# Coda-Research-Group/LearnedMetricIndex

Measured on AMD Instinct MI355X. Metric: queries/sec @ recall@10, 768-d 10M index, 10k query batch, higher is better.
Workload: dtype f16 prefilter (f32 accumulate) + f32 exact re-rank; outputs identical to the all-f32 path

## Files before the change

### learnedmetricindex_amd/csrc/lmi_front.h

```cpp
#pragma once
#include "lmi_prefilter.h"

namespace lmi {

constexpr int FR_THREADS = 1024, FR_WAVES = FR_THREADS / 64;
constexpr int FR_MAX_L = 512;
constexpr int FR_MAX_SLOTS = 1 << 17;
constexpr int FR_SLICE_G = 48;
constexpr int FR_LIST = 512;
constexpr int FP_THREADS = 512, FP_WAVES = FP_THREADS / 64;
constexpr int FR_MAX_D = 64 * 4 * 8;
static_assert(FR_SLICE_G % 2 == 0, "the 16 x 32 fragment shape pairs k16-groups");

struct FrontParams {
    const int* bucket_order;
    int nq, nb, L;
    const unsigned* epoch_dev;
    unsigned long long* gran;
    int* cb_bucket;
    int* colmap;
    RouteArrays R;
    FillRanges Z;
    const float* q;
    int d, KG16, f16x16;
// ... 207 lines not shown
                const int p = (int)(ent & 0x7fffffffu);
                const int cpos = other ? n0 + c1 + (int)__popcll(bal1 & lt) : c0 + (int)__popcll(bal0 & lt);
                P.slot_col[p] = cbs * 32 + cpos;
                P.colmap[cbs * 32 + cpos] = p / nb;
            }
            c0 += (int)__popcll(bal0);
            c1 += (int)__popcll(bal1);
        }
    }
    FR_DBG(dbg_base, 2);
}

template <int GS, int CP, bool VEC>
__global__ __launch_bounds__(FP_THREADS) void pack_kernel(FrontParams P) {
    extern __shared__ __attribute__((aligned(16))) char fp_smem[];
    __shared__ int active_s;
    const int tid = threadIdx.x, lane = tid & 63, w = __builtin_amdgcn_readfirstlane(tid >> 6);
    const int bid = blockIdx.x;
    const unsigned epoch_v = *P.epoch_dev;
    for (int r = 0; r < P.Z.count; ++r)
        for (long long i = (long long)bid * FP_THREADS + tid; i < P.Z.n[r]; i += (long long)gridDim.x * FP_THREADS) P.Z.p[r][i] = P.Z.v[r];
    for (long long p = (long long)bid * FP_THREADS + tid; p < (long long)P.nq * P.nb; p += (long long)gridDim.x * FP_THREADS) {
        const int br = P.bucket_order[p];
        if (!(br >= 0 && br < P.L && P.R.nb_rows[br] > 0)) P.slot_col[p] = -1;
    }
    if (bid == 0) {
        FR_DBG(0, 0);
        const int L = P.L;
        int* nbr = reinterpret_cast<int*>(fp_smem);
        int* m_s = nbr + fr_lpad(L);
        int* m0_s = m_s + fr_lpad(L);
// ... 9 lines not shown
        for (int o = 32; o > 0; o >>= 1) { pairs += __shfl_xor(pairs, o); items += __shfl_xor(items, o); }
        __shared__ long long red[2][FP_WAVES];
        if (lane == 0) { red[0][w] = pairs; red[1][w] = items; }
        __syncthreads();
        if (tid == 0) {
            long long ps = 0, is = 0;
            for (int i = 0; i < FP_WAVES; ++i) { ps += red[0][i]; is += red[1][i]; }
            P.R.stats[0] = ps;
            P.R.stats[1] = is;
        }
        FR_DBG(0, 1);
        RouteArrays R2 = P.R;
        R2.m = m_s;
        R2.m0 = m0_s;
        R2.nb_rows = nbr;
        route_group_body<false, FP_THREADS>(L, R2, sort_s, &active_s);
        FR_DBG(0, 4);
        return;
    }
    const unsigned long long alloc = P.gran[P.L];
    const int n_cb = (unsigned)(alloc >> 32) == epoch_v ? (int)(unsigned)alloc : 0;
    const int cb = bid - 1;
    if (cb >= n_cb) return;
    char* stage = fp_smem;
    const int b = P.cb_bucket[cb];
    const int d = P.d, KG16 = P.KG16;
    const int nchunk_row = (d + 7) >> 3;
    constexpr int CPW = 64 / GS;
    constexpr int NCOL = (32 + FP_WAVES * CPW - 1) / (FP_WAVES * CPW);
    const int gl = lane % GS, sub = lane / GS;
    const float xn = __uint_as_float(P.bnorm[b]), dx = __uint_as_float(P.bdelta[b]);
// ... 101 lines not shown
```

### learnedmetricindex_amd/csrc/lmi_hip.hip

```cpp
#include "lmi_host.h"
#include "lmi_host_model.h"
#include "lmi_host_build.h"
#include "lmi_host_mutate.h"
#include "lmi_host_scan.h"
#include "lmi_host_search.h"
#include "lmi_host_comm.h"
#include "lmi_host_debug.h"
#include <mutex>

extern "C" LMI_API int lmi_abi_version(void) { return LMI_ABI_VERSION; }
#ifndef LMI_SOURCE_SHA16
#define LMI_SOURCE_SHA16 "unknown"
#endif
#define LMI_STR2(x) #x
#define LMI_STR(x) LMI_STR2(x)
extern "C" LMI_API const char* lmi_build_info(void) {
    return "src=" LMI_SOURCE_SHA16 " p2_waves=" LMI_STR(LMI_P2_WAVES) " p2_bring=" LMI_STR(LMI_P2_BR) " pf_cap=" LMI_STR(LMI_PF_CAP);
}
extern "C" LMI_API const char* lmi_last_error(void) { return g_err.c_str(); }

extern "C" LMI_API int lmi_create(int device, lmi_index** out) {
    if (!out) return fail("lmi_create: out is NULL");
    int ndev = 0;
    HIPCHK(hipGetDeviceCount(&ndev));
// ... 24 lines not shown
            HIPCHK(hipMemcpy(&ok, d_ok, sizeof(int), hipMemcpyDeviceToHost));
            HIPCHK(hipFree(d_ok));
            cached = ok;
        }
        h->pf_hw_ok = cached == 1;
        if (!h->pf_hw_ok) h->prefilter = false;
    }
    if (const char* e = getenv("LMI_RESCORE_SIMPLE")) h->rescore_streamed = !(e[0] && e[0] != '0');
    if (const char* e = getenv("LMI_PF_NO_REDO")) h->pf_redo = !(e[0] && e[0] != '0');
    if (const char* e = getenv("LMI_PF_SMALL")) h->pf_small = !(e[0] == '0');
    if (const char* e = getenv("LMI_PF_QBOUND")) h->pf_qbound = e[0] && e[0] != '0';
    if (const char* e = getenv("LMI_PF_PRIMARY")) h->pf_primary = e[0] && e[0] != '0';
    if (const char* e = getenv("LMI_PS_WIDE")) h->ps_force_wide = e[0] == '1' ? 1 : e[0] == '0' ? 0 : -1;
    if (const char* e = getenv("LMI_FRONT")) h->use_front = !(e[0] == '0');
    if (const char* e = getenv("LMI_P2_GRADED")) h->graded_chunks = !(e[0] == '0');
    if (const char* e = getenv("LMI_P2_CHUNKS")) (void)sscanf(e, "%d,%d,%d", &h->chunk_lvl_rows[0], &h->chunk_lvl_rows[1], &h->chunk_lvl_rows[2]);
    if (const char* e = getenv("LMI_P2_CHUNK_FRAC")) (void)sscanf(e, "%f,%f", &h->chunk_frac[0], &h->chunk_frac[1]);
    if (const char* e = getenv("LMI_TAIL")) h->use_tail = e[0] == '0' ? 0 : e[0] == '2' ? 2 : 1;
    if (const char* e = getenv("LMI_FR_DEBUG")) { if (e[0] == '1') { CHK(h->fr_dbg.reserve(256)); HIPCHK(hipMemset(h->fr_dbg.p, 0, 256)); } }
    {
        int khz = 0;
        if (hipDeviceGetAttribute(&khz, hipDeviceAttributeWallClockRate, device) == hipSuccess && khz > 0) h->wall_khz = (double)khz;
    }
#define LMI_PS_ATTR(K) \
    HIPCHK(hipFuncSetAttribute(reinterpret_cast<const void*>(&pass2_small_kernel<K, false, false>), hipFuncAttributeMaxDynamicSharedMemorySize, ps_lds_bytes(K, false))); \
    HIPCHK(hipFuncSetAttribute(reinterpret_cast<const void*>(&pass2_small_kernel<K, true, false>), hipFuncAttributeMaxDynamicSharedMemorySize, ps_lds_bytes(K, false))); \
    if constexpr (ps_has_wide(K)) { \
        HIPCHK(hipFuncSetAttribute(reinterpret_cast<const void*>(&pass2_small_kernel<K, false, ps_has_wide(K)>), hipFuncAttributeMaxDynamicSharedMemorySize, ps_lds_bytes(K, true))); \
        HIPCHK(hipFuncSetAttribute(reinterpret_cast<const void*>(&pass2_small_kernel<K, true, ps_has_wide(K)>), hipFuncAttributeMaxDynamicSharedMemorySize, ps_lds_bytes(K, true))); \
    }
// ... 103 lines not shown
```

### learnedmetricindex_amd/csrc/lmi_host.h

```cpp
#pragma once
#include "lmi_kernels.h"
#include "lmi_prefilter.h"
#include "lmi_pass2.h"
#include "lmi_pass2_small.h"
#include "lmi_mlp_fused.h"
#include "lmi_rescore.h"
#include "lmi_front.h"
#include "lmi_tail.h"
#include "lmi_mutate.h"

#include <algorithm>
#include <cfloat>
#include <cstdarg>
#include <cstdio>
#include <cstring>
#include <initializer_list>
#include <string>
#include <vector>

#include "lmi_hip.h"

using namespace lmi;

namespace {
// ... 136 lines not shown
    long long ev_calls = 0;
    hipEvent_t* ev = ev_ring[0];
    bool* ev_valid = valid_ring[0];
    long long h_stats[4] = {0, 0, 0, 0};
    bool stats_pending = false;
    DevBuf ts_ring;
    unsigned ts_mask[EV_RING] = {};
    unsigned long long* ts_set = nullptr;
    double wall_khz = 100000.0;
    DevBuf fr_dbg;
    DevBuf cb_alloc, cb_bucket;
    unsigned* h_oflag = nullptr;
    int overflow_armed = 0;
    bool fr_bump_pending = false;
    int use_tail = 1;
    bool graded_chunks = true;
    int chunk_lvl_rows[3] = {0, 0, 0};
    float chunk_frac[2] = {0.16f, 0.05f};
    bool use_front = true;

    std::vector<int> h_cap_rb;
    std::vector<unsigned char> h_owned;
    std::vector<unsigned char> h_any;
    lmi_index* parent = nullptr;
    int live_clones = 0;
    int64_t mut_paths[4] = {0, 0, 0, 0};
    DevBuf mut_pos, mut_ids, mut_list, mut_keep, mut_src, mut_stage, mut_word;
};

template <class F>
// ... 96 lines not shown
```

### learnedmetricindex_amd/csrc/lmi_host_debug.h

```cpp
#pragma once
#include "lmi_host_mutate.h"

static int read_event_set(const hipEvent_t* ev, const bool* ev_valid, float* ms) {
    for (int i = 0; i < LMI_T_COUNT; ++i) ms[i] = 0.0f;
    auto span = [&](int a, int b, float* out) -> int {
        if (ev_valid[a] && ev_valid[b]) HIPCHK(hipEventElapsedTime(out, ev[a], ev[b]));
        return 0;
    };
    CHK(span(0, 1, &ms[LMI_T_INFERENCE]));
    CHK(span(1, 2, &ms[LMI_T_ROUTE]));
    CHK(span(2, 3, &ms[LMI_T_SCAN]));
    CHK(span(3, 4, &ms[LMI_T_MERGE]));
    CHK(span(2, 5, &ms[LMI_T_PF_SAMPLE]));
    CHK(span(5, 6, &ms[LMI_T_PF_EMIT]));
    CHK(span(6, 7, &ms[LMI_T_RESCORE]));
    CHK(span(7, 3, &ms[LMI_T_FALLBACK]));
    int first = ev_valid[0] ? 0 : 1;
    int last = ev_valid[4] ? 4 : 1;
    CHK(span(first, last, &ms[LMI_T_TOTAL]));
    return 0;
}

static void read_stamp_set(const lmi_index* h, const unsigned long long* v, unsigned mask, float* ms) {
    for (int i = 0; i < LMI_T_COUNT; ++i) ms[i] = 0.0f;
// ... 144 lines not shown
    if (!strcmp(name, "pf_bound")) b = &h->pf_bound;
    if (!strcmp(name, "fr_dbg")) b = &h->fr_dbg;
    if (!strcmp(name, "pf_stamps")) { b = &h->pf_bound; off = h->stamps_off; }
    if (!strcmp(name, "cand_total")) {
        if (bytes != 8 || !h->last_fast) return fail("lmi_debug_peek: cand_total is 8 bytes after a prefilter scan");
        unsigned long long* d_acc = reinterpret_cast<unsigned long long*>(h->stats.as<long long>() + 2);
        HIPCHK(hipMemsetAsync(d_acc, 0, 8, h->stream));
        sum_u32_kernel<<<64, 256, 0, h->stream>>>(h->cand_cnt.as<unsigned>(), h->last_ncols, d_acc);
        HIPCHK(hipGetLastError());
        HIPCHK(hipStreamSynchronize(h->stream));
        HIPCHK(hipMemcpy(dst, d_acc, 8, hipMemcpyDeviceToHost));
        return 0;
    }
    if (!strcmp(name, "pf_redo")) b = &h->redo;
    if (!strcmp(name, "pf_fallback")) b = &h->fb_list;
    if (!b) return fail("lmi_debug_peek: unknown buffer '%s'", name);
    if (bytes < 0 || off + (size_t)bytes > b->cap) return fail("lmi_debug_peek: %lld bytes asked of a %zu-byte buffer", (long long)bytes, b->cap);
    if (bytes) HIPCHK(hipMemcpy(dst, static_cast<char*>(b->p) + off, (size_t)bytes, hipMemcpyDeviceToHost));
    return 0;
}

extern "C" LMI_API int lmi_scan_stats(lmi_index* h, double* flops, int64_t* pairs, int64_t* items) {
    if (!h) return fail("lmi_scan_stats: NULL handle");
    CHK(set_dev(h));
    if (h->stats_pending) {
        HIPCHK(hipStreamSynchronize(h->stream));
        HIPCHK(hipMemcpy(h->h_stats, h->stats.p, 32, hipMemcpyDeviceToHost));
        h->stats_pending = false;
    }
    if (pairs) *pairs = h->h_stats[0];
// ... 5 lines not shown
```

### learnedmetricindex_amd/csrc/lmi_host_scan.h

```cpp
#pragma once
#include "lmi_host.h"

static bool rescore_is_streamed(const lmi_index* h) {
    return h->rescore_streamed && rc_waves_for(h->dp, 4) > 0 && rc_wave_lds(h->dp, 4, true) <= RC_SMALL_LDS_CAP;
}
static int rescore_group_size(int nb) { return nb % 4 == 0 ? 4 : nb % 3 == 0 ? 3 : nb % 2 == 0 ? 2 : 1; }

struct ScanPlan {
    int nq, nb, kout, L;
    long long nslots;
    long long ncb_bound;
    long long ncols;
    int max_nch;
    long long part_lists;
    bool fast;
    bool low_d;
    bool ps_wide;
    int tile_cb;
    int sample_max;
    bool qbound;
    int primary_nb;
    bool use_front;
    bool streamed;
    int G, groups, sub_cap;
// ... 77 lines not shown
    augment_norm_kernel<<<cdiv(nq, 256), 256, 0, h->stream>>>(d_qs, h->d_user, h->d, nq, h->q_aug.as<float>(), h->qn2.as<float>());
    HIPCHK(hipGetLastError());
    C.q = h->q_aug.as<float>();
    C.qn2 = h->qn2.as<float>();
    return 0;
}

static int scan_reserve(lmi_index* h, ScanCall& C) {
    const ScanPlan& P = C.P;
    const int L = P.L;
    const size_t nslots = (size_t)P.nslots, ncols = (size_t)P.ncols;
    CHK(h->m.reserve((size_t)L * 4 * 3));
    CHK(h->cb_start.reserve((L + 1) * 4));
    CHK(h->item_base.reserve((L + 1) * 4));
    CHK(h->part_base.reserve((L + 1) * 8));
    CHK(h->stats.reserve(32));
    CHK(h->head.reserve(256));
    const size_t grp_ints = (size_t)NGRP * L + 2 * (size_t)NGRP * (L + 1) + 3 * NGRP + (size_t)L;
    CHK(h->grp.reserve(grp_ints * 4));
    CHK(h->slot_local.reserve(nslots * 4));
    CHK(h->slot_col.reserve(nslots * 4));
    CHK(h->colmap.reserve(ncols * 4));
    CHK(h->col_thr.reserve(ncols * 4));
    CHK(h->qfrag.reserve((size_t)P.ncb_bound * h->KGs * 1024));
    CHK(h->part_score.reserve((size_t)P.part_lists * KPB * 4));
    CHK(h->part_row.reserve((size_t)P.part_lists * KPB * 4));
    CHK(h->rank_d.reserve(nslots * KPB * 4));
    CHK(h->rank_id.reserve(nslots * KPB * 4));

    FillRanges& Z = C.Z;
    Z.count = 0;
// ... 60 lines not shown
    R.grp_base1 = R.grp_total + NGRP;
    R.grp_total1 = R.grp_base1 + (size_t)NGRP * (L + 1);
    R.dbg = nullptr;
    R.chunk_rb = h->chunk_rows / 32;
    R.chunk_rb_b = (P.fast && h->graded_chunks) ? R.grp_total1 + NGRP : nullptr;
    const int base = h->chunk_rows;
    int rows[3] = {base, base / 2, base / 4};
    if (P.low_d) rows[0] = 2 * base;
    for (int i = 0; i < 3; ++i) {
        if (h->chunk_lvl_rows[i] > 0) rows[i] = h->chunk_lvl_rows[i];
        rows[i] = std::max(P2_TILE_ROWS, rows[i] / P2_TILE_ROWS * P2_TILE_ROWS);
        R.chunk_lvl[i] = rows[i] / 32;
    }
    R.chunk_frac[0] = h->chunk_frac[0];
    R.chunk_frac[1] = h->chunk_frac[1];
    R.tile_cb = P.tile_cb;
    R.sample_max = P.sample_max;
    R.sample_items = P.fast ? 1 : 0;
    R.primary_nb = P.primary_nb;
}

static int front_separate(lmi_index* h, ScanCall& C) {
    const ScanPlan& P = C.P;
    const RouteArrays& R = C.R;
    const int L = P.L, nslots = (int)P.nslots;
    C.Z.ts = tsp(h, ST_FRONT);
    fill_ranges_kernel<<<h->num_cus * 4, 256, 0, h->stream>>>(C.Z);
    HIPCHK(hipGetLastError());
    route_count_kernel<<<cdiv(nslots, 256), 256, 0, h->stream>>>(C.order, nslots, L, R, h->slot_local.as<int>());
    HIPCHK(hipGetLastError());
// ... 124 lines not shown
    if (S.ts_start) { S.ts_end_cell = scan_end_cell(h); (void)tsp(h, ST_SCAN1); }
    scan_kernel<<<h->num_cus * h->scan_blocks_per_cu, 256, SCAN_LDS, h->stream>>>(S);
    HIPCHK(hipGetLastError());
    CHK(record(h, 3));
    return 0;
}

static void prefilter_params(lmi_index* h, const ScanCall& C, PrefilterParams& F) {
    const RouteArrays& R = C.R;
    F.slab16 = h->slab16.as<uint4>();
    F.qfrag16 = h->qfrag16.as<uint4>();
    F.KG16 = h->KG16;
    F.L = C.P.L;
    F.chunk_rb = R.chunk_rb;
    F.chunk_rb_b = R.chunk_rb_b;
    F.tile_cb = R.tile_cb;
    F.sample_max = R.sample_max;
    F.rb_start = h->d_rb_start.as<int>();
    F.nb_rows = R.nb_rows;
    F.nch = R.nch;
    F.m = R.m;
    F.m0 = R.m0;
    F.cb_start = R.cb_start;
    F.grp_bucket = R.grp_bucket;
    F.grp_base = R.grp_base;
    F.grp_n = R.grp_n;
    F.grp_total = R.grp_total;
    F.grp_base1 = R.grp_base1;
    F.grp_total1 = R.grp_total1;
    F.ncols = C.P.ncols;
// ... 279 lines not shown
```

### learnedmetricindex_amd/csrc/lmi_kernels.h

```cpp
#pragma once
#include <hip/hip_runtime.h>
#include <stdint.h>

namespace lmi {

typedef float f32x16 __attribute__((ext_vector_type(16)));

constexpr int KPB = 10;
#ifndef LMI_SCAN_RB
#define LMI_SCAN_RB 1
#endif
constexpr int RB = LMI_SCAN_RB;
constexpr int TILE_ROWS = 128 * RB;
constexpr int TILE_COLS = 128;
constexpr int STAGE_G = 4;
constexpr int SCAN_LDS = 0;
constexpr unsigned NOROW = 0xFFFFFFFFu;
constexpr int NGRP = 8;

__device__ __forceinline__ int acc_row(int r, int h) { return (r & 3) + 8 * (r >> 2) + 4 * h; }

enum { ST_MLP0 = 0, ST_MLP1, ST_FRONT, ST_P1, ST_P2, ST_P2END, ST_TAIL, ST_FB, ST_MERGE, ST_END, ST_SCAN0, ST_SCAN1,
       ST_CLK_WALL, ST_CLK_CYC,
       ST_COUNT = 16 };
// ... 313 lines not shown
    int* grp_bucket;
    int* grp_base;
    int* grp_n;
    int* grp_total;
    int* grp_base1;
    int* grp_total1;
    int tile_cb;
    int primary_nb;
    int sample_items;
    int sample_max;
    unsigned long long* dbg;
    int* chunk_rb_b;
    int chunk_rb;
    int chunk_lvl[3];
    float chunk_frac[2];
};
__device__ __forceinline__ int chunks_of(int n_rows, int crb) { return (((n_rows + 31) >> 5) + crb - 1) / crb; }

#ifndef LMI_PF_SAMPLE_ROWS
#define LMI_PF_SAMPLE_ROWS 512
#endif
#ifndef LMI_PF_SAMPLE
#define LMI_PF_SAMPLE 16
#endif
constexpr int PF_SAMPLE = LMI_PF_SAMPLE;
#ifndef LMI_PF_SAMPLE_LOWD
#define LMI_PF_SAMPLE_LOWD 8
#endif
constexpr int PF_SAMPLE_LOWD = LMI_PF_SAMPLE_LOWD, PF_SAMPLE_LOWD_KG = 4;
__device__ __forceinline__ int sample_stride(int n_b, int smax) {
// ... 23 lines not shown
    }
    local -= g_all * nqt_all;
    const int g = local / nqt_primary;
    *qt = local - g * nqt_primary;
    *j0 = g * P1_TPI * 2 + 1;
    *nt = min(P1_TPI, n_pri - g * P1_TPI);
    return false;
}
__device__ __forceinline__ int sample_tiles256(int n_b, int smax) {
    const int nt = (((n_b + 31) >> 5) + 7) / 8;
    const int s = sample_stride(n_b, smax);
    return (nt + s - 1) / s;
}

__device__ __forceinline__ int query_tiles(int m, int tile_cb) { return (((m + 31) >> 5) + tile_cb - 1) / tile_cb; }

constexpr int ROUTE_LDS_BUCKETS = 4096;
constexpr int ROUTE_OTHER = 1 << 30;
__global__ __launch_bounds__(256) void route_count_kernel(const int* __restrict__ bucket_order, int nslots, int L,
                                                          RouteArrays R, int* __restrict__ slot_local) {
    __shared__ int cnt_s[2 * ROUTE_LDS_BUCKETS];
    const int p = blockIdx.x * blockDim.x + threadIdx.x;
    int b = -1;
    bool other = false;
    if (p < nslots) {
        b = bucket_order[p];
        if (!(b >= 0 && b < L && R.nb_rows[b] > 0)) b = -1;
        if (b >= 0 && R.primary_nb > 0) {
            const int r = p % R.primary_nb;
            for (int j = p - r; j < p; ++j) {
// ... 67 lines not shown
}

__host__ __device__ inline int route_group_pow2(int L) { int p = 64; while (p < L) p <<= 1; return p; }
__host__ __device__ inline size_t route_group_lds(int L) { return (size_t)route_group_pow2(L) * 8 + (size_t)L * 8; }
constexpr int ROUTE_MAX_BUCKETS = 8000;
constexpr int ROUTE_ID_BITS = 20;
template <bool GLOBAL, int NT = 1024>
__device__ __forceinline__ void route_group_body(int L, const RouteArrays& R, char* base, int* active_sp) {
    int& active_s = *active_sp;
    const int P = route_group_pow2(L);
    unsigned long long* key_s = reinterpret_cast<unsigned long long*>(base);
    int* items_s = reinterpret_cast<int*>(key_s + P);
    int* items1_s = items_s + L;
    int* order_s = GLOBAL ? items1_s + L : reinterpret_cast<int*>(base);
    const int t = threadIdx.x;
    if (t == 0) active_s = 0;
    __syncthreads();
    {
        int mine = 0;
        for (int b = t; b < P; b += NT) {
            unsigned long long key = ~0ull;
            if (b < L) {
                const int m = R.m[b];
                long long work = (long long)m * R.nb_rows[b];
                mine += work > 0;
                items_s[b] = query_tiles(m, R.tile_cb) * R.nch[b];
                const int mp = R.sample_items ? R.m0[b] : 0;
                items1_s[b] = (R.sample_items && m > 0) ? pass1_items(sample_tiles256(R.nb_rows[b], R.sample_max), query_tiles(m, R.tile_cb), query_tiles(mp, R.tile_cb)) : 0;
                if (work > (1ll << 43) - 1) work = (1ll << 43) - 1;
                key = ((unsigned long long)((1ll << 43) - 1 - work) << ROUTE_ID_BITS) | (unsigned long long)b;
            }
            key_s[b] = key;
        }
        if (mine) atomicAdd(&active_s, mine);
    }
    __syncthreads();
    if (R.dbg && t == 0) R.dbg[2] = wall_clock64();
    bool ranked = false;
    int my_rank[2] = {0, 0}, my_id[2] = {0, 0};
    if (!GLOBAL && P <= 2 * NT && P <= 1024) {
        ranked = true;
#pragma unroll
        for (int u = 0; u < 2; ++u) {
            const int i = t + u * NT;
            if (i < P) {
                const unsigned long long mine = key_s[i];
                int r = 0;
                long long w_all = 0, w_tail = 0;
#pragma unroll 8
                for (int o = 0; o < P; ++o) {
                    const unsigned long long ko = key_s[o];
// ... 91 lines not shown
                        R.grp_base1[g * (L + 1) + r + 1] = carry + x;
                    }
                }
                carry += __shfl(x, 63, 64);
            }
            if (ln == 0) {
                if (!second) { R.grp_n[g] = n_g; R.grp_total[g] = carry; }
                else R.grp_total1[g] = carry;
            }
        }
    }
}
template <bool GLOBAL>
__global__ __launch_bounds__(1024) void route_group_kernel(int L, RouteArrays R, char* scratch) {
    extern __shared__ __attribute__((aligned(16))) char grp_smem[];
    __shared__ int active_s;
    route_group_body<GLOBAL>(L, R, GLOBAL ? scratch : grp_smem, &active_s);
}

__global__ void route_fill_kernel(const int* __restrict__ bucket_order, const int* __restrict__ slot_local,
                                  int nslots, int nb, const int* __restrict__ cb_start, const int* __restrict__ m0,
                                  int* __restrict__ colmap, int* __restrict__ slot_col) {
    int p = blockIdx.x * blockDim.x + threadIdx.x;
    if (p >= nslots) return;
    int loc = slot_local[p];
    int col = -1;
    if (loc >= 0) {
        const int b = bucket_order[p];
        col = cb_start[b] * 32 + ((loc & ROUTE_OTHER) ? m0[b] + (loc & (ROUTE_OTHER - 1)) : loc);
        colmap[col] = p / nb;
    }
    slot_col[p] = col;
// ... 521 lines not shown
```

### learnedmetricindex_amd/csrc/lmi_pass2.h

```cpp
#pragma once
#include <type_traits>

#include "lmi_prefilter.h"

namespace lmi {

constexpr int P2_G = 2;
constexpr int P2_MAXCB = 12;
#ifndef LMI_P2_WAVES
#define LMI_P2_WAVES 8
#endif
constexpr int P2_WAVES = LMI_P2_WAVES;
static_assert(P2_WAVES == 4 || P2_WAVES == 8, "");
constexpr int P2_BLOCKS_PER_CU = 8 / P2_WAVES;
constexpr int P2_TILE_RB = 8;
constexpr int P2_TILE_ROWS = 32 * P2_TILE_RB;
constexpr int P2_SLOT_BYTES = P2_MAXCB * P2_G * 1024;
constexpr int P2_RING = 3;
constexpr int P2_NSL = 16;
constexpr int P2_NSL_BIG = 8;
static_assert(P2_NSL * 16 == P2_NSL_BIG * 32, "bound_merge2_kernel reads 256 values per column either way");
constexpr int P2_LIST = 64 + 1;
constexpr int P2_AREG0 = 232;
#define LMI_P2_NUM_VGPR_ATTR 116
// ... 15 lines not shown

#ifdef LMI_P2_STAMPS
#ifndef LMI_P2_STAMPS_SAMPLE
#define LMI_P2_STAMPS_SAMPLE 0
#endif
#define P2_STAMP(PH) if (SAMPLE == (LMI_P2_STAMPS_SAMPLE != 0)) { const unsigned long long t_ = __builtin_readcyclecounter(); st_acc[PH] += t_ - st_last; st_last = t_; }
#else
#define P2_STAMP(PH)
#endif
#if defined(LMI_P2_STAMPS) && defined(LMI_P2_STAMPS_FINE)
#define P2_STAMP_FINE(PH) P2_STAMP(PH)
#else
#define P2_STAMP_FINE(PH)
#endif

template <int NCB, bool SAMPLE>
struct Tile2 {
    static constexpr int G = P2_G;
    static constexpr int Q = G * NCB;
#ifndef LMI_P2_BR
#define LMI_P2_BR 3
#endif
    static constexpr int BR = LMI_P2_BR;
    static_assert(BR == 3 || BR == 6, "3 Q must be a multiple of BR for every NCB");
    static constexpr int D = NCB < BR - 1 ? NCB : BR - 1;
    static constexpr int PBL = (NCB + 1) / 2;
    static constexpr int PA = G;
    static_assert(G == 2, "written out for two k-groups per stage");

    const PrefilterParams& P;
    unsigned ring;
    uint4* ring_p;
    uint2* sList;
    float* sThr;
    uint4* sPend;
    int lane, w;
    unsigned lds_lane;
    typedef float f32x4v __attribute__((ext_vector_type(4)));
    f32x4v acc[NCB][2][2];
// ... 168 lines not shown
        else asm volatile("s_waitcnt vmcnt(%1)" : "+v"(pend_pos) : "n"(2 * PA) : "memory");
        if (pend_pos != 0xffffffffu) {
            u32x4 e;
            const unsigned pa = (unsigned)reinterpret_cast<uintptr_t>(sPend + w * 64) + (unsigned)ln * 16u;
            asm volatile("ds_read_b128 %0, %1\n\ts_waitcnt lgkmcnt(0)" : "=v"(e) : "v"(pa) : "memory");
            cand_store(P, (size_t)e.x, pend_pos, e.y, __uint_as_float(e.z));
        }
        pend_pos = 0xffffffffu;
    }

    __device__ __forceinline__ void epilogue_emit(int rb_tile0, int n_b, size_t col0) {
        const int ln = lane_id();
        const int quad = ln >> 4, c16 = ln & 15;
#ifdef LMI_ABL_NOEPI
#pragma unroll
        for (int n = 0; n < NCB; ++n) asm volatile("" :: "v"(acc[n][0][0]), "v"(acc[n][1][0]), "v"(acc[n][0][1]), "v"(acc[n][1][1]));
        return;
#endif
        const unsigned row0 = (unsigned)((rb_tile0 + w) * 32);
        if (row0 + 32u > (unsigned)n_b) {
            int lim = n_b - (int)row0 - 4 * quad;
#pragma unroll
            for (int n = 0; n < NCB; ++n) {
                asm volatile("" : "+v"(lim));
#pragma unroll
                for (int rh = 0; rh < 2; ++rh)
#pragma unroll
                    for (int r = 0; r < 4; ++r)
                        if (16 * rh + r >= lim) { acc[n][rh][0][r] = __builtin_nanf(""); acc[n][rh][1][r] = __builtin_nanf(""); }
            }
        }
        const unsigned list_addr = (unsigned)reinterpret_cast<uintptr_t>(sList + w * P2_LIST);
        int tot = 0;
        const unsigned kb = (unsigned)((c16 << 8) | (4 * quad));
        const unsigned thr_addr = (unsigned)reinterpret_cast<uintptr_t>(sThr) + (unsigned)c16 * 4u;
        constexpr int TB = 2;
        float thr[2][TB][2];
        auto thr_load = [&](int nb0, float (&t)[TB][2]) __attribute__((always_inline)) {
#pragma unroll
            for (int i = 0; i < TB; ++i) {
                const int n = min(nb0 + i, NCB - 1);
                asm volatile("ds_read_b32 %0, %1" : "=v"(t[i][0]) : "v"(thr_addr + (unsigned)(n * 128)) : "memory");
                asm volatile("ds_read_b32 %0, %1" : "=v"(t[i][1]) : "v"(thr_addr + (unsigned)(n * 128 + 64)) : "memory");
            }
        };
        thr_load(0, thr[0]);
#pragma unroll
        for (int n = 0; n < NCB; ++n) {
            constexpr int dummy = 0; (void)dummy;
            if (n % TB == 0) {
                asm volatile("s_waitcnt lgkmcnt(0)" ::: "memory");
#pragma unroll
                for (int i = 0; i < TB; ++i) asm volatile("" : "+v"(thr[(n / TB) & 1][i][0]), "+v"(thr[(n / TB) & 1][i][1]));
                if (n + TB < NCB) thr_load(n + TB, thr[((n / TB) + 1) & 1]);
            }
            float gm[2][2], t0, mh[2];
#pragma unroll
            for (int ch = 0; ch < 2; ++ch) {
#pragma unroll
                for (int rh = 0; rh < 2; ++rh) {
                    asm("v_max3_f32 %0, %1, %2, %3" : "=v"(t0) : "v"(acc[n][rh][ch][0]), "v"(acc[n][rh][ch][1]), "v"(acc[n][rh][ch][2]));
                    asm("v_max_f32 %0, %1, %2" : "=v"(gm[ch][rh]) : "v"(t0), "v"(acc[n][rh][ch][3]));
                }
                asm("v_max_f32 %0, %1, %2" : "=v"(mh[ch]) : "v"(gm[ch][0]), "v"(gm[ch][1]));
            }
            const float th0 = thr[(n / TB) & 1][n % TB][0], th1 = thr[(n / TB) & 1][n % TB][1];
            bool any = (mh[0] >= th0) | (mh[1] >= th1);
#ifdef LMI_ABL_NOEMIT
            any = any && th0 == 12345.678f;
#endif
            if (__builtin_expect(__ballot(any) == 0ull, 1)) continue;
#pragma unroll
            for (int ch = 0; ch < 2; ++ch) {
                const float th = ch ? th1 : th0;
#pragma unroll
                for (int rh = 0; rh < 2; ++rh) {
                    if (__ballot(gm[ch][rh] >= th) == 0ull) continue;
#pragma unroll
                    for (int r = 0; r < 4; ++r) {
                        const bool pass = acc[n][rh][ch][r] >= th;
                        const unsigned long long mask = __ballot(pass);
                        if (__builtin_expect(mask != 0ull, 0)) {
                            if (pass) {
                                const int my = tot + (int)__builtin_amdgcn_mbcnt_hi((unsigned)(mask >> 32), __builtin_amdgcn_mbcnt_lo((unsigned)mask, 0u));
                                const unsigned key = kb + (unsigned)(((n * 32 + 16 * ch) << 8) | (16 * rh + r));
                                const unsigned la = list_addr + (unsigned)min(my, 64) * 8u;
                                const unsigned sb = __float_as_uint(acc[n][rh][ch][r]);
                                const u32x2 ent = {key, sb};
// ... 16 lines not shown
                const unsigned pa = (unsigned)reinterpret_cast<uintptr_t>(sPend + w * 64) + (unsigned)ln * 16u;
                asm volatile("ds_write_b128 %0, %1" :: "v"(pa), "v"(pe) : "memory");
#ifdef LMI_ABL_NOATOMIC
                pend_pos = (unsigned)ln;
#else
                const unsigned* cnt_addr = P.cand_cnt + pcol;
                const unsigned one = 1u;
                asm volatile("global_atomic_add %0, %1, %2, off sc0" : "=v"(pend_pos) : "v"(cnt_addr), "v"(one) : "memory");
#endif
            }
        } else if (tot > 64) {
#pragma unroll
            for (int n = 0; n < NCB; ++n) {
#pragma unroll
                for (int ch = 0; ch < 2; ++ch) {
                    const float th = sThr[n * 32 + 16 * ch + c16];
                    unsigned rowq = row0 + 4u * (unsigned)quad;
                    asm volatile("" : "+v"(rowq));
#pragma unroll
                    for (int rh = 0; rh < 2; ++rh)
#pragma unroll
                        for (int r = 0; r < 4; ++r)
                            if (acc[n][rh][ch][r] >= th) {
                                const size_t col = col0 + n * 32 + 16 * ch + c16;
                                const unsigned pos = atomicAdd(P.cand_cnt + col, 1u);
                                cand_store(P, col, pos, rowq + (unsigned)(16 * rh + r), acc[n][rh][ch][r]);
                            }
                }
            }
        }
// ... 1 lines not shown

    __device__ __forceinline__ void epilogue_sample(int rb_tile0, int n_b, size_t col0, int m_left, int list_j, bool use_atomic, int rb_in_tile) {
        const int ln = lane_id();
        const int quad = ln >> 4, c16 = ln & 15;
        const unsigned row0 = (unsigned)((rb_tile0 + w) * 32);
        const bool ragged = row0 + 32u > (unsigned)n_b;
        int lim = ragged ? n_b - (int)row0 - 4 * quad : 64;
#pragma unroll
        for (int n = 0; n < NCB; ++n) {
            if (ragged) {
                asm volatile("" : "+v"(lim));
#pragma unroll
                for (int rh = 0; rh < 2; ++rh)
#pragma unroll
                    for (int r = 0; r < 4; ++r)
                        if (16 * rh + r >= lim) { acc[n][rh][0][r] = -INFINITY; acc[n][rh][1][r] = -INFINITY; }
            }
#pragma unroll
            for (int ch = 0; ch < 2; ++ch) {
                float m0, m1, m2;
                asm("v_max3_f32 %0, %1, %2, %3" : "=v"(m0) : "v"(acc[n][0][ch][0]), "v"(acc[n][0][ch][1]), "v"(acc[n][0][ch][2]));
                asm("v_max3_f32 %0, %1, %2, %3" : "=v"(m1) : "v"(acc[n][1][ch][0]), "v"(acc[n][1][ch][1]), "v"(acc[n][1][ch][2]));
                asm("v_max3_f32 %0, %1, %2, %3" : "=v"(m2) : "v"(m0), "v"(m1), "v"(acc[n][0][ch][3]));
                asm("v_max_f32 %0, %1, %2" : "=v"(m2) : "v"(m2), "v"(acc[n][1][ch][3]));
                const float mx = m2;
                if (n * 32 + 16 * ch + c16 < m_left) {
                    float* dst = P.bound + ((size_t)(list_j * 32 + (rb_in_tile + w) * 4 + quad)) * (size_t)P.ncols + (col0 + n * 32 + 16 * ch + c16);
                    if (!use_atomic) *dst = mx;
                    else {
                        if (mx >= 0.0f) atomicMax(reinterpret_cast<int*>(dst), __float_as_int(mx));
                        else atomicMin(reinterpret_cast<unsigned*>(dst), __float_as_uint(mx));
                    }
                }
            }
// ... 176 lines not shown
    const int q = blockIdx.x * blockDim.x + threadIdx.x;
    if (q >= nq) return;
    float lq = -INFINITY;
    for (int r = 0; r < nb; ++r) {
        const int col = slot_col[q * nb + r];
        if (col >= 0) lq = fmaxf(lq, bound1[col] - 0.5f * eps2[col]);
    }
    if (!(lq > -INFINITY)) return;
    lq -= fabsf(lq) * 4.8e-7f;
    for (int r = 0; r < nb; ++r) {
        const int col = slot_col[q * nb + r];
        if (col >= 0) bound1[col] = fmaxf(bound1[col], lq + 0.5f * eps2[col] * 0.9999f);
    }
}

struct P2Item { int b, cbt0, ncb_tile, ch, m_use, nt; };
template <bool SAMPLE>
__device__ __forceinline__ void p2_decode_item(const PrefilterParams& P, int b, int local, P2Item& it) {
    int qt = 0, ch = 0, nt = 1;
    bool all_cols = true;
    if (SAMPLE) {
        const int nqa = query_tiles(P.m[b], P.tile_cb), nqp = query_tiles(P.m0[b], P.tile_cb);
        all_cols = pass1_decode(local, p2_sample_tiles(P.nb_rows[b], P.sample_max), nqa, nqp, &ch, &nt, &qt);
    }
    it.nt = nt;
    it.m_use = all_cols ? P.m[b] : P.m0[b];
    const int ncb_b = (it.m_use + 31) >> 5;
    const int nqt = (ncb_b + P.tile_cb - 1) / P.tile_cb;
    const int per = (ncb_b + nqt - 1) / nqt;
    if (!SAMPLE) { qt = local % nqt; ch = local / nqt; }
    it.b = b;
    it.ch = ch;
    it.cbt0 = qt * per;
    it.ncb_tile = min(per, ncb_b - it.cbt0);
}
template <bool SAMPLE>
__device__ __forceinline__ bool p2_pop_item(const PrefilterParams& P, int& grp, int* s_item, P2Item& it) {
    if (threadIdx.x == 0) {
        int b = -1, local = 0;
        do {
            b = -1;
            unsigned* heads = P.head + (SAMPLE ? 24 : 0);
            const int* totals = SAMPLE ? P.grp_total1 : P.grp_total;
            const int* bases = SAMPLE ? P.grp_base1 : P.grp_base;
            for (int tries = 0; tries < NGRP; ++tries) {
                const int tot = totals[grp];
                if (__hip_atomic_load(&heads[grp], __ATOMIC_RELAXED, __HIP_MEMORY_SCOPE_AGENT) < (unsigned)tot) {
                    const int itn = (int)atomicAdd(&heads[grp], 1u);
                    if (itn < tot) {
// ... 97 lines not shown
    __shared__ uint2 sList[SAMPLE ? 1 : P2_WAVES * P2_LIST];
    __shared__ float sThr[SAMPLE ? 1 : P2_MAXCB * 32];
    __shared__ __attribute__((aligned(16))) uint4 sPend[SAMPLE ? 1 : P2_WAVES * 64];
    __shared__ int s_item[2];
    __shared__ int s_prefix[P2_PREFIX_CAP_K];
    __shared__ int s_gb[P2_PREFIX_CAP_K];
    if (!SAMPLE && P.redo_count && *P.redo_count == 0u) return;
    ts_first(P.ts_start);
    unsigned long long clk_w0 = 0, clk_c0 = 0;
    if (!SAMPLE) clk_begin(P.ts_end_cell ? P.ts_start : nullptr, clk_w0, clk_c0);
    P2Queue<SAMPLE, 2, 64 * P2_WAVES, P2_PREFIX_CAP_K> queue{P, s_item, s_prefix, s_gb};
    queue.init();
    P2Item item;
    while (queue.next(item)) {
        const int b = item.b, cbt0 = item.cbt0, ch = item.ch, m_use = item.m_use, nt = item.nt;
#define P2_CASE(N) case N: { Tile2<N, SAMPLE> it{P, (unsigned)reinterpret_cast<uintptr_t>(ring), ring, sList, sThr, sPend}; it.run(b, cbt0, ch, m_use, nt, queue); break; }
        switch (item.ncb_tile) {
            P2_CASE(1) P2_CASE(2) P2_CASE(3) P2_CASE(4) P2_CASE(5) P2_CASE(6)
            P2_CASE(7) P2_CASE(8) P2_CASE(9) P2_CASE(10) P2_CASE(11)
            default: { Tile2<12, SAMPLE> it{P, (unsigned)reinterpret_cast<uintptr_t>(ring), ring, sList, sThr, sPend}; it.run(b, cbt0, ch, m_use, nt, queue); break; }
        }
#undef P2_CASE
    }
    if (!SAMPLE) clk_end(P.ts_end_cell ? P.ts_start : nullptr, ST_P2, clk_w0, clk_c0);
#ifdef LMI_P2_ENDS
    if (!SAMPLE && P.ts_end_cell && threadIdx.x == 0 && blockIdx.x < 256) {
        P.stamps[192 + blockIdx.x] = wall_clock64();
        if (blockIdx.x == 0) P.stamps[191] = clk_w0;
    }
#endif
    ts_max(P.ts_end_cell);
}

}
```

### learnedmetricindex_amd/csrc/lmi_prefilter.h

```cpp
#pragma once
#include "lmi_kernels.h"


namespace lmi {

typedef _Float16 half8 __attribute__((ext_vector_type(8)));

constexpr int PF_STAGE_G = 2;
#ifndef LMI_PF_CAP
#define LMI_PF_CAP 1024
#endif
constexpr int PF_CAP = LMI_PF_CAP;
constexpr int PF_KEEP = 64;

__global__ void scatter_rows_kernel(const float* __restrict__ src, int d, const int* __restrict__ pos,
                                    long long row0, const long long* __restrict__ index, long long n_total, long long nrows,
                                    float* __restrict__ dst, int pitch) {
    const long long idx = (long long)blockIdx.x * blockDim.x + threadIdx.x;
    if (idx >= nrows * d) return;
    const long long i = idx / d;
    const int k = (int)(idx - i * d);
    const long long o = index ? index[i] : row0 + i;
    if (o < 0 || o >= n_total) return;
    const long long p = pos[o];
// ... 219 lines not shown
    unsigned* fail;
    unsigned launch;
};
__device__ __forceinline__ void pf_x_append(const OverflowLog& X, size_t col, unsigned e, unsigned row, float s) {
    const unsigned i = X.cap ? atomicAdd(X.head, 1u) : 0xffffffffu;
    if (i < X.cap) X.log[i] = make_uint4((unsigned)col, e | (X.launch << 31), row, __float_as_uint(s));
    else atomicOr(X.fail, 1u);
}

struct PrefilterParams {
    const uint4* slab16;
    const uint4* qfrag16;
    int KG16;
    int L;
    int chunk_rb;
    const int* chunk_rb_b;
    int sample_max;
    int tile_cb;
    const int* rb_start;
    const int* nb_rows;
    const int* nch;
    const int* m;
    const int* m0;
    const int* cb_start;
    const int* grp_bucket;
    const int* grp_base;
    const int* grp_n;
    const int* grp_total;
    const int* grp_base1;
    const int* grp_total1;
// ... 471 lines not shown
```

Measured before the change: 2.102 million.

## Skip the dead 16-column half of the last query block in pass-2 tiles

Pass-2 tiles now get a HALF template form. When the last 32-wide query column block of a tile holds at most 16 live queries, the unused 16-column fragment is dropped: fewer fragments (Q reduced by one) and no epilogue thresholding or emit work for those columns. The item decoder flags these tiles and the dispatch switch doubles its template instantiations to cover the half variants. This adds code size and compile time, and a routing-stage counter records how many half tiles exist, for debugging.

```diff
diff --git a/learnedmetricindex_amd/csrc/lmi_front.h b/learnedmetricindex_amd/csrc/lmi_front.h
--- a/learnedmetricindex_amd/csrc/lmi_front.h
+++ b/learnedmetricindex_amd/csrc/lmi_front.h
@@ -245,7 +245,7 @@
 template <int GS, int CP, bool VEC>
 __global__ __launch_bounds__(FP_THREADS) void pack_kernel(FrontParams P) {
     extern __shared__ __attribute__((aligned(16))) char fp_smem[];
-    __shared__ int active_s;
+    __shared__ int active_s[2];
     const int tid = threadIdx.x, lane = tid & 63, w = __builtin_amdgcn_readfirstlane(tid >> 6);
     const int bid = blockIdx.x;
     const unsigned epoch_v = *P.epoch_dev;
@@ -285,7 +285,7 @@
         R2.m = m_s;
         R2.m0 = m0_s;
         R2.nb_rows = nbr;
-        route_group_body<false, FP_THREADS>(L, R2, sort_s, &active_s);
+        route_group_body<false, FP_THREADS>(L, R2, sort_s, active_s);
         FR_DBG(0, 4);
         return;
     }
diff --git a/learnedmetricindex_amd/csrc/lmi_hip.hip b/learnedmetricindex_amd/csrc/lmi_hip.hip
--- a/learnedmetricindex_amd/csrc/lmi_hip.hip
+++ b/learnedmetricindex_amd/csrc/lmi_hip.hip
@@ -62,6 +62,7 @@
     if (const char* e = getenv("LMI_PS_WIDE")) h->ps_force_wide = e[0] == '1' ? 1 : e[0] == '0' ? 0 : -1;
     if (const char* e = getenv("LMI_FRONT")) h->use_front = !(e[0] == '0');
     if (const char* e = getenv("LMI_P2_GRADED")) h->graded_chunks = !(e[0] == '0');
+    if (const char* e = getenv("LMI_P2_HALFCB")) h->half_cb = !(e[0] == '0');
     if (const char* e = getenv("LMI_P2_CHUNKS")) (void)sscanf(e, "%d,%d,%d", &h->chunk_lvl_rows[0], &h->chunk_lvl_rows[1], &h->chunk_lvl_rows[2]);
     if (const char* e = getenv("LMI_P2_CHUNK_FRAC")) (void)sscanf(e, "%f,%f", &h->chunk_frac[0], &h->chunk_frac[1]);
     if (const char* e = getenv("LMI_TAIL")) h->use_tail = e[0] == '0' ? 0 : e[0] == '2' ? 2 : 1;
diff --git a/learnedmetricindex_amd/csrc/lmi_host.h b/learnedmetricindex_amd/csrc/lmi_host.h
--- a/learnedmetricindex_amd/csrc/lmi_host.h
+++ b/learnedmetricindex_amd/csrc/lmi_host.h
@@ -174,6 +174,7 @@
     int overflow_armed = 0;
     bool fr_bump_pending = false;
     int use_tail = 1;
+    bool half_cb = true;
     bool graded_chunks = true;
     int chunk_lvl_rows[3] = {0, 0, 0};
     float chunk_frac[2] = {0.16f, 0.05f};
diff --git a/learnedmetricindex_amd/csrc/lmi_host_debug.h b/learnedmetricindex_amd/csrc/lmi_host_debug.h
--- a/learnedmetricindex_amd/csrc/lmi_host_debug.h
+++ b/learnedmetricindex_amd/csrc/lmi_host_debug.h
@@ -182,6 +182,7 @@
     }
     if (!strcmp(name, "pf_redo")) b = &h->redo;
     if (!strcmp(name, "pf_fallback")) b = &h->fb_list;
+    if (!strcmp(name, "p2_half_tiles")) { b = &h->stats; off = 32; }
     if (!b) return fail("lmi_debug_peek: unknown buffer '%s'", name);
     if (bytes < 0 || off + (size_t)bytes > b->cap) return fail("lmi_debug_peek: %lld bytes asked of a %zu-byte buffer", (long long)bytes, b->cap);
     if (bytes) HIPCHK(hipMemcpy(dst, static_cast<char*>(b->p) + off, (size_t)bytes, hipMemcpyDeviceToHost));
diff --git a/learnedmetricindex_amd/csrc/lmi_host_scan.h b/learnedmetricindex_amd/csrc/lmi_host_scan.h
--- a/learnedmetricindex_amd/csrc/lmi_host_scan.h
+++ b/learnedmetricindex_amd/csrc/lmi_host_scan.h
@@ -115,7 +115,7 @@
     CHK(h->cb_start.reserve((L + 1) * 4));
     CHK(h->item_base.reserve((L + 1) * 4));
     CHK(h->part_base.reserve((L + 1) * 8));
-    CHK(h->stats.reserve(32));
+    CHK(h->stats.reserve(48));
     CHK(h->head.reserve(256));
     const size_t grp_ints = (size_t)NGRP * L + 2 * (size_t)NGRP * (L + 1) + 3 * NGRP + (size_t)L;
     CHK(h->grp.reserve(grp_ints * 4));
@@ -206,6 +206,8 @@
     }
     R.chunk_frac[0] = h->chunk_frac[0];
     R.chunk_frac[1] = h->chunk_frac[1];
+    R.half_cb = (P.fast && !P.low_d && h->half_cb) ? 1 : 0;
+    R.half_tiles = reinterpret_cast<unsigned*>(h->stats.as<long long>() + 4);
     R.tile_cb = P.tile_cb;
     R.sample_max = P.sample_max;
     R.sample_items = P.fast ? 1 : 0;
@@ -360,6 +362,7 @@
     F.L = C.P.L;
     F.chunk_rb = R.chunk_rb;
     F.chunk_rb_b = R.chunk_rb_b;
+    F.half_cb = R.half_cb;
     F.tile_cb = R.tile_cb;
     F.sample_max = R.sample_max;
     F.rb_start = h->d_rb_start.as<int>();
diff --git a/learnedmetricindex_amd/csrc/lmi_kernels.h b/learnedmetricindex_amd/csrc/lmi_kernels.h
--- a/learnedmetricindex_amd/csrc/lmi_kernels.h
+++ b/learnedmetricindex_amd/csrc/lmi_kernels.h
@@ -351,6 +351,8 @@
     int chunk_rb;
     int chunk_lvl[3];
     float chunk_frac[2];
+    int half_cb;
+    unsigned* half_tiles;
 };
 __device__ __forceinline__ int chunks_of(int n_rows, int crb) { return (((n_rows + 31) >> 5) + crb - 1) / crb; }
 
@@ -404,6 +406,8 @@
 }
 
 __device__ __forceinline__ int query_tiles(int m, int tile_cb) { return (((m + 31) >> 5) + tile_cb - 1) / tile_cb; }
+__device__ __forceinline__ bool p2_half_tile(int m_use, int cbt0, int ncb_tile) { return m_use - (cbt0 + ncb_tile - 1) * 32 <= 16; }
+__device__ __forceinline__ int p2_half_tiles_of(int m) { return (m > 0 && ((m - 1) & 31) < 16) ? 1 : 0; }
 
 constexpr int ROUTE_LDS_BUCKETS = 4096;
 constexpr int ROUTE_OTHER = 1 << 30;
@@ -501,16 +505,18 @@
     int* items1_s = items_s + L;
     int* order_s = GLOBAL ? items1_s + L : reinterpret_cast<int*>(base);
     const int t = threadIdx.x;
-    if (t == 0) active_s = 0;
+    int& half_s = active_sp[1];
+    if (t == 0) { active_s = 0; half_s = 0; }
     __syncthreads();
     {
-        int mine = 0;
+        int mine = 0, mine_half = 0;
         for (int b = t; b < P; b += NT) {
             unsigned long long key = ~0ull;
             if (b < L) {
                 const int m = R.m[b];
                 long long work = (long long)m * R.nb_rows[b];
                 mine += work > 0;
+                if (R.half_cb && work > 0) mine_half += p2_half_tiles_of(m);
                 items_s[b] = query_tiles(m, R.tile_cb) * R.nch[b];
                 const int mp = R.sample_items ? R.m0[b] : 0;
                 items1_s[b] = (R.sample_items && m > 0) ? pass1_items(sample_tiles256(R.nb_rows[b], R.sample_max), query_tiles(m, R.tile_cb), query_tiles(mp, R.tile_cb)) : 0;
@@ -520,8 +526,10 @@
             key_s[b] = key;
         }
         if (mine) atomicAdd(&active_s, mine);
+        if (mine_half) atomicAdd(&half_s, mine_half);
     }
     __syncthreads();
+    if (R.half_tiles && t == 0) *R.half_tiles = (unsigned)half_s;
     if (R.dbg && t == 0) R.dbg[2] = wall_clock64();
     bool ranked = false;
     int my_rank[2] = {0, 0}, my_id[2] = {0, 0};
@@ -643,8 +651,8 @@
 template <bool GLOBAL>
 __global__ __launch_bounds__(1024) void route_group_kernel(int L, RouteArrays R, char* scratch) {
     extern __shared__ __attribute__((aligned(16))) char grp_smem[];
-    __shared__ int active_s;
-    route_group_body<GLOBAL>(L, R, GLOBAL ? scratch : grp_smem, &active_s);
+    __shared__ int active_s[2];
+    route_group_body<GLOBAL>(L, R, GLOBAL ? scratch : grp_smem, active_s);
 }
 
 __global__ void route_fill_kernel(const int* __restrict__ bucket_order, const int* __restrict__ slot_local,
diff --git a/learnedmetricindex_amd/csrc/lmi_pass2.h b/learnedmetricindex_amd/csrc/lmi_pass2.h
--- a/learnedmetricindex_amd/csrc/lmi_pass2.h
+++ b/learnedmetricindex_amd/csrc/lmi_pass2.h
@@ -53,15 +53,17 @@
 #define P2_STAMP_FINE(PH)
 #endif
 
-template <int NCB, bool SAMPLE>
+template <int NCB, bool HALF, bool SAMPLE>
 struct Tile2 {
     static constexpr int G = P2_G;
-    static constexpr int Q = G * NCB;
+    static constexpr int Q = G * NCB - (HALF ? 1 : 0);
+    static constexpr bool live(int n, int ch) { return !(HALF && n == NCB - 1 && ch == 1); }
 #ifndef LMI_P2_BR
 #define LMI_P2_BR 3
 #endif
     static constexpr int BR = LMI_P2_BR;
     static_assert(BR == 3 || BR == 6, "3 Q must be a multiple of BR for every NCB");
+    static_assert((3 * Q) % BR == 0, "the half form's odd Q closes a ring of three only");
     static constexpr int D = NCB < BR - 1 ? NCB : BR - 1;
     static constexpr int PBL = (NCB + 1) / 2;
     static constexpr int PA = G;
@@ -260,7 +262,10 @@
         const int quad = ln >> 4, c16 = ln & 15;
 #ifdef LMI_ABL_NOEPI
 #pragma unroll
-        for (int n = 0; n < NCB; ++n) asm volatile("" :: "v"(acc[n][0][0]), "v"(acc[n][1][0]), "v"(acc[n][0][1]), "v"(acc[n][1][1]));
+        for (int n = 0; n < NCB; ++n) {
+            asm volatile("" :: "v"(acc[n][0][0]), "v"(acc[n][1][0]));
+            if (live(n, 1)) asm volatile("" :: "v"(acc[n][0][1]), "v"(acc[n][1][1]));
+        }
         return;
 #endif
         const unsigned row0 = (unsigned)((rb_tile0 + w) * 32);
@@ -273,7 +278,7 @@
                 for (int rh = 0; rh < 2; ++rh)
 #pragma unroll
                     for (int r = 0; r < 4; ++r)
-                        if (16 * rh + r >= lim) { acc[n][rh][0][r] = __builtin_nanf(""); acc[n][rh][1][r] = __builtin_nanf(""); }
+                        if (16 * rh + r >= lim) { acc[n][rh][0][r] = __builtin_nanf(""); if (live(n, 1)) acc[n][rh][1][r] = __builtin_nanf(""); }
             }
         }
         const unsigned list_addr = (unsigned)reinterpret_cast<uintptr_t>(sList + w * P2_LIST);
@@ -303,6 +308,7 @@
             float gm[2][2], t0, mh[2];
 #pragma unroll
             for (int ch = 0; ch < 2; ++ch) {
+                if (!live(n, ch)) continue;
 #pragma unroll
                 for (int rh = 0; rh < 2; ++rh) {
                     asm("v_max3_f32 %0, %1, %2, %3" : "=v"(t0) : "v"(acc[n][rh][ch][0]), "v"(acc[n][rh][ch][1]), "v"(acc[n][rh][ch][2]));
@@ -311,13 +317,15 @@
                 asm("v_max_f32 %0, %1, %2" : "=v"(mh[ch]) : "v"(gm[ch][0]), "v"(gm[ch][1]));
             }
             const float th0 = thr[(n / TB) & 1][n % TB][0], th1 = thr[(n / TB) & 1][n % TB][1];
-            bool any = (mh[0] >= th0) | (mh[1] >= th1);
+            bool any = mh[0] >= th0;
+            if (live(n, 1)) any |= mh[1] >= th1;
 #ifdef LMI_ABL_NOEMIT
             any = any && th0 == 12345.678f;
 #endif
             if (__builtin_expect(__ballot(any) == 0ull, 1)) continue;
 #pragma unroll
             for (int ch = 0; ch < 2; ++ch) {
+                if (!live(n, ch)) continue;
                 const float th = ch ? th1 : th0;
 #pragma unroll
                 for (int rh = 0; rh < 2; ++rh) {
@@ -364,6 +372,7 @@
             for (int n = 0; n < NCB; ++n) {
 #pragma unroll
                 for (int ch = 0; ch < 2; ++ch) {
+                    if (!live(n, ch)) continue;
                     const float th = sThr[n * 32 + 16 * ch + c16];
                     unsigned rowq = row0 + 4u * (unsigned)quad;
                     asm volatile("" : "+v"(rowq));
@@ -395,10 +404,11 @@
                 for (int rh = 0; rh < 2; ++rh)
 #pragma unroll
                     for (int r = 0; r < 4; ++r)
-                        if (16 * rh + r >= lim) { acc[n][rh][0][r] = -INFINITY; acc[n][rh][1][r] = -INFINITY; }
+                        if (16 * rh + r >= lim) { acc[n][rh][0][r] = -INFINITY; if (live(n, 1)) acc[n][rh][1][r] = -INFINITY; }
             }
 #pragma unroll
             for (int ch = 0; ch < 2; ++ch) {
+                if (!live(n, ch)) continue;
                 float m0, m1, m2;
                 asm("v_max3_f32 %0, %1, %2, %3" : "=v"(m0) : "v"(acc[n][0][ch][0]), "v"(acc[n][0][ch][1]), "v"(acc[n][0][ch][2]));
                 asm("v_max3_f32 %0, %1, %2, %3" : "=v"(m1) : "v"(acc[n][1][ch][0]), "v"(acc[n][1][ch][1]), "v"(acc[n][1][ch][2]));
@@ -605,7 +615,7 @@
     }
 }
 
-struct P2Item { int b, cbt0, ncb_tile, ch, m_use, nt; };
+struct P2Item { int b, cbt0, ncb_tile, ch, m_use, nt, half; };
 template <bool SAMPLE>
 __device__ __forceinline__ void p2_decode_item(const PrefilterParams& P, int b, int local, P2Item& it) {
     int qt = 0, ch = 0, nt = 1;
@@ -624,6 +634,7 @@
     it.ch = ch;
     it.cbt0 = qt * per;
     it.ncb_tile = min(per, ncb_b - it.cbt0);
+    it.half = (P.half_cb && p2_half_tile(it.m_use, it.cbt0, it.ncb_tile)) ? 1 : 0;
 }
 template <bool SAMPLE>
 __device__ __forceinline__ bool p2_pop_item(const PrefilterParams& P, int& grp, int* s_item, P2Item& it) {
@@ -751,12 +762,15 @@
     P2Item item;
     while (queue.next(item)) {
         const int b = item.b, cbt0 = item.cbt0, ch = item.ch, m_use = item.m_use, nt = item.nt;
-#define P2_CASE(N) case N: { Tile2<N, SAMPLE> it{P, (unsigned)reinterpret_cast<uintptr_t>(ring), ring, sList, sThr, sPend}; it.run(b, cbt0, ch, m_use, nt, queue); break; }
-        switch (item.ncb_tile) {
-            P2_CASE(1) P2_CASE(2) P2_CASE(3) P2_CASE(4) P2_CASE(5) P2_CASE(6)
-            P2_CASE(7) P2_CASE(8) P2_CASE(9) P2_CASE(10) P2_CASE(11)
-            default: { Tile2<12, SAMPLE> it{P, (unsigned)reinterpret_cast<uintptr_t>(ring), ring, sList, sThr, sPend}; it.run(b, cbt0, ch, m_use, nt, queue); break; }
-        }
+#define P2_TILE(H) { Tile2<(H + 1) / 2, (H & 1) != 0, SAMPLE> it{P, (unsigned)reinterpret_cast<uintptr_t>(ring), ring, sList, sThr, sPend}; it.run(b, cbt0, ch, m_use, nt, queue); break; }
+#define P2_CASE(H) case H: P2_TILE(H)
+        switch (2 * item.ncb_tile - item.half) {
+            P2_CASE(1) P2_CASE(2) P2_CASE(3) P2_CASE(4) P2_CASE(5) P2_CASE(6) P2_CASE(7) P2_CASE(8)
+            P2_CASE(9) P2_CASE(10) P2_CASE(11) P2_CASE(12) P2_CASE(13) P2_CASE(14) P2_CASE(15) P2_CASE(16)
+            P2_CASE(17) P2_CASE(18) P2_CASE(19) P2_CASE(20) P2_CASE(21) P2_CASE(22) P2_CASE(23)
+            default: P2_TILE(24)
+        }
+#undef P2_TILE
 #undef P2_CASE
     }
     if (!SAMPLE) clk_end(P.ts_end_cell ? P.ts_start : nullptr, ST_P2, clk_w0, clk_c0);
diff --git a/learnedmetricindex_amd/csrc/lmi_prefilter.h b/learnedmetricindex_amd/csrc/lmi_prefilter.h
--- a/learnedmetricindex_amd/csrc/lmi_prefilter.h
+++ b/learnedmetricindex_amd/csrc/lmi_prefilter.h
@@ -257,6 +257,7 @@
     int KG16;
     int L;
     int chunk_rb;
+    int half_cb;
     const int* chunk_rb_b;
     int sample_max;
     int tile_cb;
```

Result: no change. 2.084 million (-0.8%).
